# codex-storage/codex-storage-proofs-circuits

Hardware: AMD Instinct MI355X
Metric: Poseidon2-BN254 permutations/sec per GPU; full proof-input witnesses/sec (higher is better)
Workload: dtype u32x9 (29-bit limbs, Montgomery mod BN254 r)

## Files before the change

### codex-storage-proofs-circuits_amd/csrc/proof_many.cpp

```cpp
#include <hip/hip_runtime.h>

#include <fcntl.h>
#include <unistd.h>

#include <algorithm>
#include <cstring>
#include <map>
#include <memory>
#include <string>
#include <vector>

#include "dataset_obj.hpp"
#include "proof_input_obj.hpp"
#include "trees.hpp"

using namespace cp2i;

namespace {

struct Req {
  cp2_dataset* ds = nullptr;
  uint64_t slot = 0;
  uint8_t entropy[32];
  size_t at = 0;
  size_t id = 0;
};

int refuse(cp2_ctx* ctx, size_t i, const std::string& why) {
  ctx->err = "request " + std::to_string(i) + ": " + why;
  return CP2_ERR_INVALID;
}

size_t depth_of(size_t n) { return layer_sizes_of(n).size() - 1; }

bool same_circuit(const cp2_config& a, const cp2_config& b) {
  return a.max_depth == b.max_depth && a.max_log2_nslots == b.max_log2_nslots && a.cell_size == b.cell_size && a.block_size == b.block_size &&
         a.n_samples == b.n_samples;
}

int validate(cp2_ctx* ctx, cp2_dataset* const* ds, const uint64_t* slot_idx, size_t n) {
  for (size_t i = 0; i < n; ++i) {
    const cp2_dataset* d = ds[i];
    if (!d) return refuse(ctx, i, "NULL dataset");
    if (d->ctx != ctx) return refuse(ctx, i, "its dataset belongs to another context");
    const cp2_config& c = d->cfg;
    if (!same_circuit(c, ds[0]->cfg))
      return refuse(ctx, i, "its circuit parameters (maxDepth, maxLog2NSlots, cellSize, blockSize, nSamples) differ from request 0's");
    const uint64_t s = slot_idx[i];
    if (s < d->first_slot || s - d->first_slot >= d->n_local)
      return refuse(ctx, i, "slot " + std::to_string(s) + " is not local to its dataset (slots " + std::to_string(d->first_slot) + " .. " +
                                std::to_string(d->first_slot + d->n_local - 1) + ")");
    if (!d->have_roots && !(d->first_slot == 0 && d->n_local == c.n_slots))
      return refuse(ctx, i, "its dataset has no dataset tree: not all of its slots are local and cp2_dataset_set_roots was never called");
    if (!is_pow2(c.n_cells) || (c.n_samples && c.n_cells < 2))
      return refuse(ctx, i, "nCells " + std::to_string(c.n_cells) + " is not a power of two >= 2");
    const size_t cpb = c.block_size / c.cell_size;
    if (depth_of(cpb) + depth_of(c.n_cells / cpb) > (size_t)c.max_depth)
      return refuse(ctx, i, "its slot tree is deeper than maxDepth");
    if (depth_of(c.n_slots) > (size_t)c.max_log2_nslots)
      return refuse(ctx, i, "its dataset tree is deeper than maxLog2NSlots");
    if (!d->trees && d->tree_mode == 2 && d->csizes.size() - 1 != depth_of(c.n_cells / cpb))
      return refuse(ctx, i, "its compact layers do not match its configuration");
  }
  return CP2_OK;
}

int check_roots(cp2_ctx* ctx, cp2_dataset* const* ds, const uint64_t* slot_idx, size_t n) {
  std::vector<uint64_t> a(n);
  for (size_t i = 0; i < n; ++i)
    a[i] = (uint64_t)reinterpret_cast<uintptr_t>(dataset_roots_dev(ds[i])) + (slot_idx[i] - ds[i]->first_slot) * 32;
  std::vector<uint8_t> got(n * 32);
  DevBuf d_a, d_r;
  CP2_TRY(d_a.scratch(ctx, n * 8));
  CP2_TRY(d_r.scratch(ctx, n * 32));
  CP2_HIP(ctx, hipMemcpyAsync(d_a.p, a.data(), n * 8, hipMemcpyHostToDevice, ctx->stream));
  CP2_HIP(ctx, cp2k::launch_gather_addr(static_cast<const uint64_t*>(d_a.p), n, 32, d_r.p, ctx->stream));
  CP2_HIP(ctx, hipMemcpyAsync(got.data(), d_r.p, n * 32, hipMemcpyDeviceToHost, ctx->stream));
  CP2_HIP(ctx, hipStreamSynchronize(ctx->stream));
  for (size_t i = 0; i < n; ++i)
    if (std::memcmp(&got[i * 32], &ds[i]->dlayers[slot_idx[i] * 32], 32) != 0)
      return refuse(ctx, i, "the root its dataset tree holds for slot " + std::to_string(slot_idx[i]) +
                                " (cp2_dataset_set_roots) differs from the slot's built root");
  return CP2_OK;
}

int prepare(cp2_ctx* ctx, cp2_dataset* const* ds, const uint64_t* slot_idx, size_t n) {
  CP2_TRY(validate(ctx, ds, slot_idx, n));
  CP2_HIP(ctx, hipSetDevice(ctx->device));
  for (size_t i = 0; i < n; ++i)
    if (!ds[i]->have_roots) CP2_TRY(cp2_dataset_set_roots(ds[i], nullptr));
  return check_roots(ctx, ds, slot_idx, n);
}

std::string who(bool named, const Req* r) { return named ? "request " + std::to_string(r->id) + ": " : std::string(); }

int run_pass(cp2_ctx* ctx, const std::vector<const Req*>& rq, size_t n_rf, size_t n_rfile, size_t n_cf, bool named, cp2_proof_input** out) {
  const size_t n = rq.size(), nr = n_rf + n_rfile;
  const cp2_config& c0 = rq[0]->ds->cfg;
  const size_t ns = c0.n_samples, md = (size_t)c0.max_depth, cs = c0.cell_size, bs = c0.block_size, cpb = bs / cs;
  const size_t T = n * ns, R = nr * ns, C = T - R, RF = n_rf * ns, CF = n_cf * ns;
  auto store = std::make_shared<BatchStore>();
  if (T) {
    std::vector<cp2k::ManyReq> reqs(n);
    std::vector<cp2k::TreeGeom> geoms;
    std::map<std::string, uint32_t> geom_of;
    for (size_t j = 0; j < n; ++j) {
      const cp2_dataset* ds = rq[j]->ds;
      cp2k::ManyReq& q = reqs[j];
      std::memset(&q, 0, sizeof q);
      std::memcpy(q.entropy, rq[j]->entropy, 32);
      std::memcpy(q.slot_root, &ds->dlayers[rq[j]->slot * 32], 32);
      q.n_cells = ds->cfg.n_cells;
      q.cpb = cpb;
      if (j < nr) {
        cp2k::TreeGeom g;
        std::memset(&g, 0, sizeof g);
        trees_geom(ds->trees, &g);
        auto it = geom_of.emplace(std::string(reinterpret_cast<const char*>(&g), sizeof g), (uint32_t)geoms.size());
        if (it.second) geoms.push_back(g);
        q.geom = it.first->second;
        q.nodes = (uint64_t)reinterpret_cast<uintptr_t>(ds->trees->nodes.p);
        q.slot = rq[j]->slot - ds->first_slot;
      }
    }
    std::vector<uint64_t> blk(C), gen, cpaths, ctail, ccell;
    std::vector<uint8_t> checks(2 * C * 32);
    PinBuf h_blocks;
    const size_t rows = T * md + T + 2 * C;
    DevBuf d_req, d_geom, d_idx, d_blk, d_addr, d_rows, d_cells, d_gen, d_caddr;
    CP2_TRY(d_req.scratch(ctx, n * sizeof(cp2k::ManyReq)));
    CP2_TRY(d_geom.scratch(ctx, std::max<size_t>(1, geoms.size()) * sizeof(cp2k::TreeGeom)));
    CP2_TRY(d_idx.scratch(ctx, T * 8));
    CP2_TRY(d_blk.scratch(ctx, T * 8));
    CP2_TRY(d_addr.scratch(ctx, rows * 8));
    CP2_TRY(d_rows.scratch(ctx, rows * 32));
    CP2_TRY(d_cells.scratch(ctx, (C * cpb + T) * cs));
    CP2_TRY(store->idx.alloc(ctx, T * 8));
    CP2_TRY(store->paths.alloc(ctx, T * md * 32));
    CP2_TRY(store->leaves.alloc(ctx, T * 32));
    CP2_TRY(store->cells.alloc(ctx, T * cs));
    uint8_t* cells_out = d_cells.u8() + C * cpb * cs;
    uint64_t* addr = static_cast<uint64_t*>(d_addr.p);
    CP2_HIP(ctx, hipMemcpyAsync(d_req.p, reqs.data(), n * sizeof(cp2k::ManyReq), hipMemcpyHostToDevice, ctx->stream));
    if (!geoms.empty())
      CP2_HIP(ctx, hipMemcpyAsync(d_geom.p, geoms.data(), geoms.size() * sizeof(cp2k::TreeGeom), hipMemcpyHostToDevice, ctx->stream));
    CP2_HIP(ctx, cp2k::launch_sample_many(static_cast<const cp2k::ManyReq*>(d_req.p), static_cast<const cp2k::TreeGeom*>(d_geom.p), n,
                                          (uint32_t)ns, (uint32_t)md, static_cast<uint64_t*>(d_idx.p), static_cast<uint64_t*>(d_blk.p), addr,
                                          ctx->stream));
    CP2_HIP(ctx, hipMemcpyAsync(store->idx.p, d_idx.p, T * 8, hipMemcpyDeviceToHost, ctx->stream));
    if (C) CP2_HIP(ctx, hipMemcpyAsync(blk.data(), static_cast<uint64_t*>(d_blk.p) + R, C * 8, hipMemcpyDeviceToHost, ctx->stream));
    CP2_HIP(ctx, hipStreamSynchronize(ctx->stream));
    const uint64_t* idx = static_cast<const uint64_t*>(store->idx.p);

    gen.assign((CF + RF) * 2, 0);
    uint64_t* seeds = gen.data();
    uint64_t* firsts = seeds + CF + RF;
    for (size_t q = 0; q < CF; ++q) {
      const Req* r = rq[nr + q / ns];
      seeds[q] = cp2_slot_seed(r->ds->cfg.seed, r->slot);
      firsts[q] = blk[q] * cpb;
    }
    for (size_t p = 0; p < RF; ++p) {
      const Req* r = rq[p / ns];
      seeds[CF + p] = cp2_slot_seed(r->ds->cfg.seed, r->slot);
      firsts[CF + p] = idx[p];
    }
    if (CF + RF) {
      CP2_TRY(d_gen.scratch(ctx, gen.size() * 8));
      const uint64_t* dg = static_cast<const uint64_t*>(d_gen.p);
      CP2_HIP(ctx, hipMemcpyAsync(d_gen.p, gen.data(), gen.size() * 8, hipMemcpyHostToDevice, ctx->stream));
      CP2_HIP(ctx, cp2k::launch_gen_fake_cells_many(dg, dg + CF + RF, cpb, CF * cpb, cs, d_cells.p, ctx->stream));
      CP2_HIP(ctx, cp2k::launch_gen_fake_cells_many(dg + CF, dg + CF + RF + CF, 1, RF, cs, cells_out, ctx->stream));
    }
    if (C > CF) {
      const size_t n_req_file = (C - CF) / ns;
      CP2_TRY(h_blocks.alloc(ctx, (C - CF) * bs));
      std::vector<std::string> failed(fill_threads(ctx));
      on_threads(fill_threads(ctx), n_req_file, [&](int w, size_t k) {
        const size_t q0 = CF + k * ns;
        const Req* r = rq[nr + q0 / ns];
        const std::string fname = slot_file_name(r->ds->file_base, r->slot);
        const int fd = open(fname.c_str(), O_RDONLY);
        if (fd < 0) { failed[w] = who(named, r) + "slot " + std::to_string(r->slot) + ": " + slot_file_error(fname, 0); return false; }
        int err = 0;
        size_t c = 0;
        for (; c < ns && !err; ++c) err = slot_file_read_rest(fd, h_blocks.u8() + (q0 - CF + c) * bs, bs, blk[q0 + c] * bs);
        close(fd);
        if (err) {
          failed[w] = who(named, r) + "block " + std::to_string(blk[q0 + c - 1]) + " of slot " + std::to_string(r->slot) +
                      ": " + slot_file_error(fname, err);
          return false;
        }
        return true;
      });
      for (const auto& f : failed)
        if (!f.empty()) { ctx->err = f; return CP2_ERR_IO; }
      CP2_HIP(ctx, hipMemcpyAsync(d_cells.u8() + CF * bs, h_blocks.p, (C - CF) * bs, hipMemcpyHostToDevice, ctx->stream));
    }
    cp2_slot_trees* mini = nullptr;
    struct Mini { cp2_slot_trees*& t; ~Mini() { cp2_slot_trees_free(t); } } mini_guard{mini};
    if (C) {
      cpaths.assign(C * md, 0);
      ctail.assign(3 * C, 0);
      ccell.assign(C, 0);
      CP2_TRY(cp2_slot_trees_build_dev(ctx, d_cells.p, C, cs, bs, cpb, &mini));
      const size_t depth_b = depth_of(cpb);
      const uint64_t mb = (uint64_t)reinterpret_cast<uintptr_t>(mini->nodes.p);
      std::vector<uint64_t> rr(depth_b + 1);
      for (size_t q = 0; q < C; ++q) {
        const Req* r = rq[nr + q / ns];
        const cp2_dataset* ds = r->ds;
        const uint64_t ls = r->slot - ds->first_slot, cell = idx[R + q], b = blk[q], in_block = cell % cpb;
        const uint64_t kb = (uint64_t)reinterpret_cast<uintptr_t>(ds->compact.p);
        uint64_t* P = &cpaths[q * md];
        path_rows(mini, q, in_block, depth_b + 1, rr.data());
        for (size_t d = 0; d < depth_b; ++d) P[d] = rr[d] == NO_ROW ? 0 : mb + rr[d] * 32;
        uint64_t j = b, m = ds->cfg.n_cells / cpb;
        for (size_t d = 0; d + 1 < ds->csizes.size(); ++d) {
          const uint64_t sib = j ^ 1;
          P[depth_b + d] = sib < m ? kb + (ds->coff[d] + ls * ds->csizes[d] + sib) * 32 : 0;
          j >>= 1;
          m = (m + 1) >> 1;
        }
        ctail[q] = mb + (q * cpb + in_block) * 32;
        ctail[C + 2 * q] = kb + (ds->coff[0] + ls * ds->csizes[0] + b) * 32;
        ctail[C + 2 * q + 1] = mb + (mini->toff[0] + q) * 32;
        ccell[q] = (uint64_t)reinterpret_cast<uintptr_t>(d_cells.u8()) + (q * cpb + in_block) * cs;
      }
      CP2_TRY(d_caddr.scratch(ctx, C * 8));
      CP2_HIP(ctx, hipMemcpyAsync(addr + R * md, cpaths.data(), C * md * 8, hipMemcpyHostToDevice, ctx->stream));
      CP2_HIP(ctx, hipMemcpyAsync(addr + T * md + R, ctail.data(), 3 * C * 8, hipMemcpyHostToDevice, ctx->stream));
      CP2_HIP(ctx, hipMemcpyAsync(d_caddr.p, ccell.data(), C * 8, hipMemcpyHostToDevice, ctx->stream));
      CP2_HIP(ctx, cp2k::launch_gather_addr(static_cast<const uint64_t*>(d_caddr.p), C, cs, cells_out + R * cs, ctx->stream));
    }
    CP2_HIP(ctx, cp2k::launch_gather_addr(addr, rows, 32, d_rows.p, ctx->stream));
    CP2_HIP(ctx, hipMemcpyAsync(store->paths.p, d_rows.p, T * md * 32, hipMemcpyDeviceToHost, ctx->stream));
    CP2_HIP(ctx, hipMemcpyAsync(store->leaves.p, d_rows.u8() + T * md * 32, T * 32, hipMemcpyDeviceToHost, ctx->stream));
    if (C) CP2_HIP(ctx, hipMemcpyAsync(checks.data(), d_rows.u8() + (T * md + T) * 32, 2 * C * 32, hipMemcpyDeviceToHost, ctx->stream));
    CP2_HIP(ctx, hipMemcpyAsync(store->cells.p, cells_out, T * cs, hipMemcpyDeviceToHost, ctx->stream));
    CP2_HIP(ctx, hipStreamSynchronize(ctx->stream));
    for (size_t q = 0; q < C; ++q)
      if (std::memcmp(&checks[2 * q * 32], &checks[(2 * q + 1) * 32], 32) != 0) {
        const Req* r = rq[nr + q / ns];
        ctx->err = who(named, r) + "block " + std::to_string(blk[q]) + " of slot " + std::to_string(r->slot) +
                   " does not hash to its stored root (slot data changed since the build?)";
        return CP2_ERR_IO;
      }
    if (R > RF) {
      std::vector<std::string> failed(fill_threads(ctx));
      on_threads(fill_threads(ctx), n_rfile, [&](int w, size_t k) {
        const Req* r = rq[n_rf + k];
        const std::string fname = slot_file_name(r->ds->file_base, r->slot);
        const int fd = open(fname.c_str(), O_RDONLY);
        if (fd < 0) { failed[w] = who(named, r) + slot_file_error(fname, 0); return false; }
        int err = 0;
        const size_t p0 = (n_rf + k) * ns;
        for (size_t c = 0; c < ns && !err; ++c) err = read_file_cell(fd, cs, idx[p0 + c], store->cells.u8() + (p0 + c) * cs);
        close(fd);
        if (err) { failed[w] = who(named, r) + slot_file_error(fname, err); return false; }
        return true;
      });
      for (const auto& f : failed)
        if (!f.empty()) { ctx->err = f; return CP2_ERR_IO; }
    }
  }
  std::vector<ProofItem> items(n);
  for (size_t j = 0; j < n; ++j) items[j] = {rq[j]->ds, rq[j]->slot, rq[j]->entropy, &out[rq[j]->at]};
  return proof_inputs_from_store(items.data(), n, store, store->cells.u8());
}

}

int cp2i::prove_requests(cp2_ctx* ctx, cp2_dataset* const* ds, const uint64_t* slot_idx, const uint8_t* entropies, size_t n, size_t at0,
                         bool named, cp2_proof_input** out) {
  for (size_t i = 0; i < n; ++i) out[i] = nullptr;
  if (n == 0) return CP2_OK;
  CP2_HIP(ctx, hipSetDevice(ctx->device));
  std::vector<Req> req(n);
  std::vector<const Req*> res_fake, res_file, cmp_fake, cmp_file, roots_only;
  for (size_t i = 0; i < n; ++i) {
    req[i].ds = ds[i];
    req[i].slot = slot_idx[i];
    req[i].at = i;
    req[i].id = at0 + i;
    canonical_felt(entropies + 32 * i, req[i].entropy);
    const cp2_dataset* d = ds[i];
    (d->trees ? (d->from_file ? res_file : res_fake) : d->tree_mode == 2 ? (d->from_file ? cmp_file : cmp_fake) : roots_only).push_back(&req[i]);
  }
  auto fail = [&](int st) {
    for (size_t i = 0; i < n; ++i) { cp2_proof_input_free(out[i]); out[i] = nullptr; }
    return st;
  };
  for (const Req* r : roots_only) {
    const int st = cp2_proof_inputs_generate_batch(r->ds, &r->slot, 1, r->entropy, &out[r->at]);
    if (st != CP2_OK) {
      ctx->err = who(named, r) + ctx->err;
      return fail(st);
    }
  }
  const cp2_config& c0 = ds[0]->cfg;
  const size_t per_req = std::max<size_t>(1, (size_t)c0.n_samples * c0.block_size);
  const size_t chunk = std::max<size_t>(1, ctx->stage_bytes / per_req);
  std::vector<const Req*> compact(cmp_fake);
  compact.insert(compact.end(), cmp_file.begin(), cmp_file.end());
  const size_t n_res = res_fake.size() + res_file.size();
  size_t c = 0;
  for (bool first = true; first ? n_res + compact.size() > 0 : c < compact.size(); first = false) {
    std::vector<const Req*> rq;
    if (first) {
      rq = res_fake;
      rq.insert(rq.end(), res_file.begin(), res_file.end());
    }
    const size_t c1 = std::min(compact.size(), c + chunk);
    rq.insert(rq.end(), compact.begin() + (long)c, compact.begin() + (long)c1);
    const size_t n_cf = c < cmp_fake.size() ? std::min(c1, cmp_fake.size()) - c : 0;
    const int st = run_pass(ctx, rq, first ? res_fake.size() : 0, first ? res_file.size() : 0, n_cf, named, out);
    if (st != CP2_OK) return fail(st);
    c = c1;
  }
  return CP2_OK;
}

extern "C" int cp2_proof_inputs_generate_many(cp2_ctx* ctx, cp2_dataset* const* ds, const uint64_t* slot_idx, const uint8_t* entropies, size_t n,
                                              cp2_proof_input** out) try {
  if (!ctx) return CP2_ERR_INVALID;
  if (n && (!ds || !slot_idx || !entropies || !out)) {
    ctx->err = "cp2_proof_inputs_generate_many: NULL array";
    return CP2_ERR_INVALID;
  }
  for (size_t i = 0; i < n; ++i) out[i] = nullptr;
  if (n == 0) return CP2_OK;
  CP2_REFUSE_STUCK(ctx);
  CP2_TRY(prepare(ctx, ds, slot_idx, n));
  return prove_requests(ctx, ds, slot_idx, entropies, n, 0, true, out);
} catch (const std::bad_alloc&) {
  return CP2_ERR_ALLOC;
} catch (...) {
  return CP2_ERR_INVALID;
}

extern "C" int cp2_proof_inputs_export_many(cp2_ctx* ctx, cp2_dataset* const* ds, const uint64_t* slot_idx, const uint8_t* entropies, size_t n,
                                            const char* const* paths, int threads, size_t batch, uint64_t* total_bytes) try {
  if (!ctx) return CP2_ERR_INVALID;
  if (n && (!ds || !slot_idx || !entropies)) {
    ctx->err = "cp2_proof_inputs_export_many: NULL array";
    return CP2_ERR_INVALID;
  }
  if (total_bytes) *total_bytes = 0;
  if (n == 0) return CP2_OK;
  CP2_REFUSE_STUCK(ctx);
  CP2_TRY(prepare(ctx, ds, slot_idx, n));
  if (batch == 0) batch = 512;
  if (threads < 1) threads = 1;
  uint64_t bytes = 0;
  int status = CP2_OK;
  std::vector<cp2_proof_input*> cur, next;
  auto generate = [&](size_t b0, std::vector<cp2_proof_input*>& o) -> int {
    const size_t m = std::min(batch, n - b0);
    o.assign(m, nullptr);
    return prove_requests(ctx, ds + b0, slot_idx + b0, entropies + 32 * b0, m, b0, true, o.data());
  };
  struct Release {
    std::vector<cp2_proof_input*>& v;
    ~Release() { for (auto* p : v) cp2_proof_input_free(p); v.clear(); }
  } rel_cur{cur}, rel_next{next};
  status = generate(0, cur);
  for (size_t b0 = 0; status == CP2_OK && b0 < n; b0 += batch) {
    const size_t b1 = b0 + batch;
    int gen_status = CP2_OK, st = CP2_OK;
    uint64_t got = 0;
    {
      Workers producer(1);
      if (b1 < n) producer.submit([&] { gen_status = generate(b1, next); });
      st = cp2_proof_inputs_write_json_batch(cur.data(), cur.size(), paths ? paths + b0 : nullptr, threads, &got);
    }
    bytes += got;
    for (auto* p : cur) cp2_proof_input_free(p);
    cur.clear();
    if (st != CP2_OK) status = st;
    else if (gen_status != CP2_OK) status = gen_status;
    cur.swap(next);
  }
  if (total_bytes) *total_bytes = bytes;
  return status;
} catch (const std::bad_alloc&) {
  return CP2_ERR_ALLOC;
} catch (...) {
  return CP2_ERR_INVALID;
}
```

Measured before the change: 767.1 million.

## Deduplicate touched blocks per request and double-buffer compact proof passes

Sampling now runs once for all requests. A per-request hash table then deduplicates the blocks each compact request touches, so every distinct block is read, generated and hashed only once, and pass sizing follows the distinct-block count. Passes use two preallocated device and pinned buffer sets so the host work for the next pass (file reads, path assembly) overlaps the current pass's GPU work. The cost is more code, larger and more complex buffer management, and a fallback to a single buffer set when allocation fails.

```diff
diff --git a/codex-storage-proofs-circuits_amd/csrc/proof_many.cpp b/codex-storage-proofs-circuits_amd/csrc/proof_many.cpp
--- a/codex-storage-proofs-circuits_amd/csrc/proof_many.cpp
+++ b/codex-storage-proofs-circuits_amd/csrc/proof_many.cpp
@@ -4,6 +4,9 @@
 #include <unistd.h>
 
 #include <algorithm>
+#include <chrono>
+#include <cstdio>
+#include <cstdlib>
 #include <cstring>
 #include <map>
 #include <memory>
@@ -12,6 +15,7 @@
 
 #include "dataset_obj.hpp"
 #include "proof_input_obj.hpp"
+#include "touched_plan.hpp"
 #include "trees.hpp"
 
 using namespace cp2i;
@@ -94,180 +98,313 @@
 
 std::string who(bool named, const Req* r) { return named ? "request " + std::to_string(r->id) + ": " : std::string(); }
 
-int run_pass(cp2_ctx* ctx, const std::vector<const Req*>& rq, size_t n_rf, size_t n_rfile, size_t n_cf, bool named, cp2_proof_input** out) {
-  const size_t n = rq.size(), nr = n_rf + n_rfile;
-  const cp2_config& c0 = rq[0]->ds->cfg;
-  const size_t ns = c0.n_samples, md = (size_t)c0.max_depth, cs = c0.cell_size, bs = c0.block_size, cpb = bs / cs;
-  const size_t T = n * ns, R = nr * ns, C = T - R, RF = n_rf * ns, CF = n_cf * ns;
-  auto store = std::make_shared<BatchStore>();
-  if (T) {
-    std::vector<cp2k::ManyReq> reqs(n);
-    std::vector<cp2k::TreeGeom> geoms;
-    std::map<std::string, uint32_t> geom_of;
-    for (size_t j = 0; j < n; ++j) {
-      const cp2_dataset* ds = rq[j]->ds;
-      cp2k::ManyReq& q = reqs[j];
-      std::memset(&q, 0, sizeof q);
-      std::memcpy(q.entropy, rq[j]->entropy, 32);
-      std::memcpy(q.slot_root, &ds->dlayers[rq[j]->slot * 32], 32);
-      q.n_cells = ds->cfg.n_cells;
-      q.cpb = cpb;
-      if (j < nr) {
-        cp2k::TreeGeom g;
-        std::memset(&g, 0, sizeof g);
-        trees_geom(ds->trees, &g);
-        auto it = geom_of.emplace(std::string(reinterpret_cast<const char*>(&g), sizeof g), (uint32_t)geoms.size());
-        if (it.second) geoms.push_back(g);
-        q.geom = it.first->second;
-        q.nodes = (uint64_t)reinterpret_cast<uintptr_t>(ds->trees->nodes.p);
-        q.slot = rq[j]->slot - ds->first_slot;
+struct PassDims {
+  size_t r0 = 0, r1 = 0;
+  size_t R = 0, RF = 0;
+  size_t C = 0;
+  size_t d0 = 0, D = 0, DF = 0;
+};
+
+struct PassLayout {
+  size_t n_rows = 0, root_row = 0, node_rows = 0;
+  size_t addr = 0, rows = 0, cells = 0, nodes = 0, gen = 0, caddr = 0, dev_bytes = 0;
+  size_t h_addr = 0, h_gen = 0, h_caddr = 0, h_checks = 0, h_blocks = 0, pin_bytes = 0;
+};
+
+size_t carve(size_t& off, size_t bytes) {
+  const size_t at = off;
+  off += (bytes + 255) & ~(size_t)255;
+  return at;
+}
+
+struct PassSet {
+  DevBuf dev;
+  PinBuf pin;
+  hipEvent_t done = nullptr;
+  ~PassSet() { if (done) (void)hipEventDestroy(done); }
+};
+
+struct Pass {
+  PassDims d;
+  PassLayout l;
+  std::shared_ptr<BatchStore> store;
+};
+
+struct Call {
+  cp2_ctx* ctx = nullptr;
+  bool named = false;
+  cp2_proof_input** out = nullptr;
+  std::vector<const Req*> rq;
+  size_t n_rf = 0, n_rfile = 0, n_cf = 0, n_cfile = 0;
+  size_t ns = 0, md = 0, cs = 0, bs = 0, cpb = 0;
+  std::vector<size_t> bsizes;
+  size_t per_block = 0;
+  size_t R_all = 0, C_all = 0;
+  DevBuf dev;
+  PinBuf pin;
+  uint64_t* d_raddr = nullptr;
+  uint8_t* d_rrows = nullptr;
+  const uint64_t* idx = nullptr;
+  const uint64_t* blk = nullptr;
+  TouchedPlan plan;
+  PassSet sets[2];
+  size_t nr() const { return n_rf + n_rfile; }
+  const Req* compact_req(size_t r) const { return rq[nr() + r]; }
+};
+
+PassLayout layout_of(const Call& c, const PassDims& d) {
+  PassLayout l;
+  const size_t T = d.R + d.C;
+  l.n_rows = d.C * c.md + d.C + 2 * d.D;
+  l.root_row = d.D * c.per_block;
+  l.node_rows = l.root_row + d.D;
+  size_t off = 0;
+  l.addr = carve(off, l.n_rows * 8);
+  l.rows = carve(off, l.n_rows * 32);
+  l.cells = carve(off, (d.D * c.cpb + T) * c.cs);
+  l.nodes = carve(off, l.node_rows * 32);
+  l.gen = carve(off, 2 * (d.DF + d.RF) * 8);
+  l.caddr = carve(off, d.C * 8);
+  l.dev_bytes = off;
+  off = 0;
+  l.h_addr = carve(off, l.n_rows * 8);
+  l.h_gen = carve(off, 2 * (d.DF + d.RF) * 8);
+  l.h_caddr = carve(off, d.C * 8);
+  l.h_checks = carve(off, 2 * d.D * 32);
+  l.h_blocks = carve(off, (d.D - d.DF) * c.bs);
+  l.pin_bytes = off;
+  return l;
+}
+
+int sample_all(Call& c) {
+  cp2_ctx* ctx = c.ctx;
+  const size_t n = c.rq.size(), nr = c.nr(), T_all = c.R_all + c.C_all, raddr_rows = c.R_all * c.md + c.R_all;
+  std::vector<cp2k::TreeGeom> geoms;
+  std::map<std::string, uint32_t> geom_of;
+  size_t off = 0;
+  const size_t o_req = carve(off, n * sizeof(cp2k::ManyReq)), o_idx = carve(off, T_all * 8), o_blk = carve(off, c.C_all * 8);
+  CP2_TRY(c.pin.alloc(ctx, off));
+  cp2k::ManyReq* reqs = reinterpret_cast<cp2k::ManyReq*>(c.pin.u8() + o_req);
+  for (size_t j = 0; j < n; ++j) {
+    const cp2_dataset* ds = c.rq[j]->ds;
+    cp2k::ManyReq& q = reqs[j];
+    std::memset(&q, 0, sizeof q);
+    std::memcpy(q.entropy, c.rq[j]->entropy, 32);
+    std::memcpy(q.slot_root, &ds->dlayers[c.rq[j]->slot * 32], 32);
+    q.n_cells = ds->cfg.n_cells;
+    q.cpb = c.cpb;
+    if (j < nr) {
+      cp2k::TreeGeom g;
+      std::memset(&g, 0, sizeof g);
+      trees_geom(ds->trees, &g);
+      auto it = geom_of.emplace(std::string(reinterpret_cast<const char*>(&g), sizeof g), (uint32_t)geoms.size());
+      if (it.second) geoms.push_back(g);
+      q.geom = it.first->second;
+      q.nodes = (uint64_t)reinterpret_cast<uintptr_t>(ds->trees->nodes.p);
+      q.slot = c.rq[j]->slot - ds->first_slot;
+    }
+  }
+  size_t doff = 0;
+  const size_t d_req = carve(doff, n * sizeof(cp2k::ManyReq)), d_geom = carve(doff, geoms.size() * sizeof(cp2k::TreeGeom)),
+               d_idx = carve(doff, T_all * 8), d_blk = carve(doff, c.C_all * 8), d_raddr = carve(doff, raddr_rows * 8),
+               d_rrows = carve(doff, raddr_rows * 32);
+  CP2_TRY(c.dev.scratch(ctx, doff));
+  uint8_t* base = c.dev.u8();
+  c.d_raddr = reinterpret_cast<uint64_t*>(base + d_raddr);
+  c.d_rrows = base + d_rrows;
+  const cp2k::ManyReq* dreq = reinterpret_cast<const cp2k::ManyReq*>(base + d_req);
+  uint64_t* didx = reinterpret_cast<uint64_t*>(base + d_idx);
+  CP2_HIP(ctx, hipMemcpyAsync(base + d_req, reqs, n * sizeof(cp2k::ManyReq), hipMemcpyHostToDevice, ctx->stream));
+  if (!geoms.empty())
+    CP2_HIP(ctx, hipMemcpyAsync(base + d_geom, geoms.data(), geoms.size() * sizeof(cp2k::TreeGeom), hipMemcpyHostToDevice, ctx->stream));
+  CP2_HIP(ctx, cp2k::launch_sample_many(dreq, reinterpret_cast<const cp2k::TreeGeom*>(base + d_geom), nr, (uint32_t)c.ns, (uint32_t)c.md, didx,
+                                        nullptr, c.d_raddr, ctx->stream));
+  CP2_HIP(ctx, cp2k::launch_sample_many(dreq + nr, nullptr, n - nr, (uint32_t)c.ns, (uint32_t)c.md, didx + c.R_all,
+                                        reinterpret_cast<uint64_t*>(base + d_blk), nullptr, ctx->stream));
+  if (T_all) CP2_HIP(ctx, hipMemcpyAsync(c.pin.u8() + o_idx, didx, T_all * 8, hipMemcpyDeviceToHost, ctx->stream));
+  if (c.C_all) CP2_HIP(ctx, hipMemcpyAsync(c.pin.u8() + o_blk, base + d_blk, c.C_all * 8, hipMemcpyDeviceToHost, ctx->stream));
+  CP2_HIP(ctx, hipStreamSynchronize(ctx->stream));
+  c.idx = reinterpret_cast<const uint64_t*>(c.pin.u8() + o_idx);
+  c.blk = reinterpret_cast<const uint64_t*>(c.pin.u8() + o_blk);
+  const size_t cap_blocks = ctx->stage_bytes / c.bs;
+  const size_t chunk = std::max<size_t>(1, ctx->stage_bytes / std::max<size_t>(1, c.ns * c.bs));
+  c.plan = touched_plan(c.blk, c.n_cf + c.n_cfile, c.ns, cap_blocks, 4 * chunk);
+  return CP2_OK;
+}
+
+int enqueue_pass(Call& c, Pass& p, PassSet& set) {
+  cp2_ctx* ctx = c.ctx;
+  const PassDims& d = p.d;
+  const PassLayout& l = p.l;
+  const size_t ns = c.ns, md = c.md, cs = c.cs, bs = c.bs, cpb = c.cpb, T = d.R + d.C;
+  uint8_t* dev = set.dev.u8();
+  uint8_t* pin = set.pin.u8();
+  uint8_t* d_cells = dev + l.cells;
+  uint8_t* cells_out = d_cells + d.D * cpb * cs;
+  uint8_t* d_rows = dev + l.rows;
+  uint64_t* d_addr = reinterpret_cast<uint64_t*>(dev + l.addr);
+  p.store = std::make_shared<BatchStore>();
+  CP2_TRY(p.store->idx.alloc(ctx, T * 8));
+  CP2_TRY(p.store->paths.alloc(ctx, T * md * 32));
+  CP2_TRY(p.store->leaves.alloc(ctx, T * 32));
+  CP2_TRY(p.store->cells.alloc(ctx, T * cs));
+  uint64_t* sidx = static_cast<uint64_t*>(p.store->idx.p);
+  std::memcpy(sidx, c.idx, d.R * 8);
+  std::memcpy(sidx + d.R, c.idx + c.R_all + d.r0 * ns, d.C * 8);
+  if (d.DF + d.RF) {
+    uint64_t* seeds = reinterpret_cast<uint64_t*>(pin + l.h_gen);
+    uint64_t* firsts = seeds + d.DF + d.RF;
+    for (size_t r = d.r0, k = 0; r < d.r1 && r < c.n_cf; ++r) {
+      const Req* rq = c.compact_req(r);
+      const uint64_t seed = cp2_slot_seed(rq->ds->cfg.seed, rq->slot);
+      for (size_t g = c.plan.first[r]; g < c.plan.first[r + 1]; ++g, ++k) {
+        seeds[k] = seed;
+        firsts[k] = c.plan.block[g] * cpb;
       }
     }
-    std::vector<uint64_t> blk(C), gen, cpaths, ctail, ccell;
-    std::vector<uint8_t> checks(2 * C * 32);
-    PinBuf h_blocks;
-    const size_t rows = T * md + T + 2 * C;
-    DevBuf d_req, d_geom, d_idx, d_blk, d_addr, d_rows, d_cells, d_gen, d_caddr;
-    CP2_TRY(d_req.scratch(ctx, n * sizeof(cp2k::ManyReq)));
-    CP2_TRY(d_geom.scratch(ctx, std::max<size_t>(1, geoms.size()) * sizeof(cp2k::TreeGeom)));
-    CP2_TRY(d_idx.scratch(ctx, T * 8));
-    CP2_TRY(d_blk.scratch(ctx, T * 8));
-    CP2_TRY(d_addr.scratch(ctx, rows * 8));
-    CP2_TRY(d_rows.scratch(ctx, rows * 32));
-    CP2_TRY(d_cells.scratch(ctx, (C * cpb + T) * cs));
-    CP2_TRY(store->idx.alloc(ctx, T * 8));
-    CP2_TRY(store->paths.alloc(ctx, T * md * 32));
-    CP2_TRY(store->leaves.alloc(ctx, T * 32));
-    CP2_TRY(store->cells.alloc(ctx, T * cs));
-    uint8_t* cells_out = d_cells.u8() + C * cpb * cs;
-    uint64_t* addr = static_cast<uint64_t*>(d_addr.p);
-    CP2_HIP(ctx, hipMemcpyAsync(d_req.p, reqs.data(), n * sizeof(cp2k::ManyReq), hipMemcpyHostToDevice, ctx->stream));
-    if (!geoms.empty())
-      CP2_HIP(ctx, hipMemcpyAsync(d_geom.p, geoms.data(), geoms.size() * sizeof(cp2k::TreeGeom), hipMemcpyHostToDevice, ctx->stream));
-    CP2_HIP(ctx, cp2k::launch_sample_many(static_cast<const cp2k::ManyReq*>(d_req.p), static_cast<const cp2k::TreeGeom*>(d_geom.p), n,
-                                          (uint32_t)ns, (uint32_t)md, static_cast<uint64_t*>(d_idx.p), static_cast<uint64_t*>(d_blk.p), addr,
-                                          ctx->stream));
-    CP2_HIP(ctx, hipMemcpyAsync(store->idx.p, d_idx.p, T * 8, hipMemcpyDeviceToHost, ctx->stream));
-    if (C) CP2_HIP(ctx, hipMemcpyAsync(blk.data(), static_cast<uint64_t*>(d_blk.p) + R, C * 8, hipMemcpyDeviceToHost, ctx->stream));
-    CP2_HIP(ctx, hipStreamSynchronize(ctx->stream));
-    const uint64_t* idx = static_cast<const uint64_t*>(store->idx.p);
-
-    gen.assign((CF + RF) * 2, 0);
-    uint64_t* seeds = gen.data();
-    uint64_t* firsts = seeds + CF + RF;
-    for (size_t q = 0; q < CF; ++q) {
-      const Req* r = rq[nr + q / ns];
-      seeds[q] = cp2_slot_seed(r->ds->cfg.seed, r->slot);
-      firsts[q] = blk[q] * cpb;
-    }
-    for (size_t p = 0; p < RF; ++p) {
-      const Req* r = rq[p / ns];
-      seeds[CF + p] = cp2_slot_seed(r->ds->cfg.seed, r->slot);
-      firsts[CF + p] = idx[p];
-    }
-    if (CF + RF) {
-      CP2_TRY(d_gen.scratch(ctx, gen.size() * 8));
-      const uint64_t* dg = static_cast<const uint64_t*>(d_gen.p);
-      CP2_HIP(ctx, hipMemcpyAsync(d_gen.p, gen.data(), gen.size() * 8, hipMemcpyHostToDevice, ctx->stream));
-      CP2_HIP(ctx, cp2k::launch_gen_fake_cells_many(dg, dg + CF + RF, cpb, CF * cpb, cs, d_cells.p, ctx->stream));
-      CP2_HIP(ctx, cp2k::launch_gen_fake_cells_many(dg + CF, dg + CF + RF + CF, 1, RF, cs, cells_out, ctx->stream));
-    }
-    if (C > CF) {
-      const size_t n_req_file = (C - CF) / ns;
-      CP2_TRY(h_blocks.alloc(ctx, (C - CF) * bs));
-      std::vector<std::string> failed(fill_threads(ctx));
-      on_threads(fill_threads(ctx), n_req_file, [&](int w, size_t k) {
-        const size_t q0 = CF + k * ns;
-        const Req* r = rq[nr + q0 / ns];
-        const std::string fname = slot_file_name(r->ds->file_base, r->slot);
-        const int fd = open(fname.c_str(), O_RDONLY);
-        if (fd < 0) { failed[w] = who(named, r) + "slot " + std::to_string(r->slot) + ": " + slot_file_error(fname, 0); return false; }
-        int err = 0;
-        size_t c = 0;
-        for (; c < ns && !err; ++c) err = slot_file_read_rest(fd, h_blocks.u8() + (q0 - CF + c) * bs, bs, blk[q0 + c] * bs);
-        close(fd);
-        if (err) {
-          failed[w] = who(named, r) + "block " + std::to_string(blk[q0 + c - 1]) + " of slot " + std::to_string(r->slot) +
-                      ": " + slot_file_error(fname, err);
-          return false;
-        }
-        return true;
-      });
-      for (const auto& f : failed)
-        if (!f.empty()) { ctx->err = f; return CP2_ERR_IO; }
-      CP2_HIP(ctx, hipMemcpyAsync(d_cells.u8() + CF * bs, h_blocks.p, (C - CF) * bs, hipMemcpyHostToDevice, ctx->stream));
-    }
-    cp2_slot_trees* mini = nullptr;
-    struct Mini { cp2_slot_trees*& t; ~Mini() { cp2_slot_trees_free(t); } } mini_guard{mini};
-    if (C) {
-      cpaths.assign(C * md, 0);
-      ctail.assign(3 * C, 0);
-      ccell.assign(C, 0);
-      CP2_TRY(cp2_slot_trees_build_dev(ctx, d_cells.p, C, cs, bs, cpb, &mini));
-      const size_t depth_b = depth_of(cpb);
-      const uint64_t mb = (uint64_t)reinterpret_cast<uintptr_t>(mini->nodes.p);
-      std::vector<uint64_t> rr(depth_b + 1);
-      for (size_t q = 0; q < C; ++q) {
-        const Req* r = rq[nr + q / ns];
-        const cp2_dataset* ds = r->ds;
-        const uint64_t ls = r->slot - ds->first_slot, cell = idx[R + q], b = blk[q], in_block = cell % cpb;
-        const uint64_t kb = (uint64_t)reinterpret_cast<uintptr_t>(ds->compact.p);
-        uint64_t* P = &cpaths[q * md];
-        path_rows(mini, q, in_block, depth_b + 1, rr.data());
-        for (size_t d = 0; d < depth_b; ++d) P[d] = rr[d] == NO_ROW ? 0 : mb + rr[d] * 32;
-        uint64_t j = b, m = ds->cfg.n_cells / cpb;
-        for (size_t d = 0; d + 1 < ds->csizes.size(); ++d) {
+    for (size_t q = 0; q < d.RF; ++q) {
+      const Req* rq = c.rq[q / ns];
+      seeds[d.DF + q] = cp2_slot_seed(rq->ds->cfg.seed, rq->slot);
+      firsts[d.DF + q] = c.idx[q];
+    }
+    const uint64_t* dg = reinterpret_cast<const uint64_t*>(dev + l.gen);
+    CP2_HIP(ctx, hipMemcpyAsync(dev + l.gen, seeds, 2 * (d.DF + d.RF) * 8, hipMemcpyHostToDevice, ctx->stream));
+    CP2_HIP(ctx, cp2k::launch_gen_fake_cells_many(dg, dg + d.DF + d.RF, cpb, d.DF * cpb, cs, d_cells, ctx->stream));
+    CP2_HIP(ctx, cp2k::launch_gen_fake_cells_many(dg + d.DF, dg + d.DF + d.RF + d.DF, 1, d.RF, cs, cells_out, ctx->stream));
+  }
+  if (d.D > d.DF) {
+    const size_t f0 = std::max(d.r0, c.n_cf), g0 = d.d0 + d.DF;
+    uint8_t* h_blocks = pin + l.h_blocks;
+    std::vector<std::string> failed(fill_threads(ctx));
+    on_threads(fill_threads(ctx), d.r1 - f0, [&](int w, size_t k) {
+      const size_t r = f0 + k;
+      const Req* rq = c.compact_req(r);
+      const std::string fname = slot_file_name(rq->ds->file_base, rq->slot);
+      const int fd = open(fname.c_str(), O_RDONLY);
+      if (fd < 0) { failed[w] = who(c.named, rq) + "slot " + std::to_string(rq->slot) + ": " + slot_file_error(fname, 0); return false; }
+      int err = 0;
+      size_t g = c.plan.first[r];
+      for (; g < c.plan.first[r + 1] && !err; ++g) err = slot_file_read_rest(fd, h_blocks + (g - g0) * bs, bs, c.plan.block[g] * bs);
+      close(fd);
+      if (err) {
+        failed[w] = who(c.named, rq) + "block " + std::to_string(c.plan.block[g - 1]) + " of slot " + std::to_string(rq->slot) +
+                    ": " + slot_file_error(fname, err);
+        return false;
+      }
+      return true;
+    });
+    for (const auto& f : failed)
+      if (!f.empty()) { ctx->err = f; return CP2_ERR_IO; }
+    CP2_HIP(ctx, hipMemcpyAsync(d_cells + d.DF * bs, h_blocks, (d.D - d.DF) * bs, hipMemcpyHostToDevice, ctx->stream));
+  }
+  if (d.D) {
+    uint8_t* nodes = dev + l.nodes;
+    const uint64_t mb = (uint64_t)reinterpret_cast<uintptr_t>(nodes);
+    const size_t nb = c.bsizes.size(), depth_b = nb - 1;
+    std::vector<size_t> boff(nb, 0);
+    for (size_t k = 1; k < nb; ++k) boff[k] = boff[k - 1] + d.D * c.bsizes[k - 1];
+    CP2_HIP(ctx, cp2k::launch_hash_cells(d_cells, cs, d.D * cpb, nodes, ctx->stream));
+    for (size_t k = 0; k + 1 < nb; ++k)
+      CP2_HIP(ctx, cp2k::launch_compress_layer(nodes + boff[k] * 32, nodes + boff[k + 1] * 32, c.bsizes[k], d.D, k == 0, c.bsizes[k],
+                                               c.bsizes[k + 1], ctx->stream));
+    uint64_t* h_addr = reinterpret_cast<uint64_t*>(pin + l.h_addr);
+    uint64_t* h_leaf = h_addr + d.C * md;
+    uint64_t* h_check = h_leaf + d.C;
+    uint64_t* h_caddr = reinterpret_cast<uint64_t*>(pin + l.h_caddr);
+    std::memset(h_addr, 0, d.C * md * 8);
+    for (size_t r = d.r0; r < d.r1; ++r) {
+      const Req* rq = c.compact_req(r);
+      const cp2_dataset* ds = rq->ds;
+      const uint64_t ls = rq->slot - ds->first_slot, kb = (uint64_t)reinterpret_cast<uintptr_t>(ds->compact.p);
+      for (size_t g = c.plan.first[r]; g < c.plan.first[r + 1]; ++g) {
+        h_check[2 * (g - d.d0)] = kb + (ds->coff[0] + ls * ds->csizes[0] + c.plan.block[g]) * 32;
+        h_check[2 * (g - d.d0) + 1] = mb + (boff[depth_b] + (g - d.d0)) * 32;
+      }
+      for (size_t s = 0; s < ns; ++s) {
+        const size_t lane = r * ns + s, q = lane - d.r0 * ns, g = c.plan.lane_pair[lane] - d.d0;
+        const uint64_t cell = c.idx[c.R_all + lane], b = c.blk[lane], in_block = cell % cpb;
+        uint64_t* P = h_addr + q * md;
+        uint64_t j = in_block, m = cpb;
+        for (size_t k = 0; k < depth_b; ++k) {
           const uint64_t sib = j ^ 1;
-          P[depth_b + d] = sib < m ? kb + (ds->coff[d] + ls * ds->csizes[d] + sib) * 32 : 0;
+          P[k] = sib < m ? mb + (boff[k] + g * c.bsizes[k] + sib) * 32 : 0;
           j >>= 1;
           m = (m + 1) >> 1;
         }
-        ctail[q] = mb + (q * cpb + in_block) * 32;
-        ctail[C + 2 * q] = kb + (ds->coff[0] + ls * ds->csizes[0] + b) * 32;
-        ctail[C + 2 * q + 1] = mb + (mini->toff[0] + q) * 32;
-        ccell[q] = (uint64_t)reinterpret_cast<uintptr_t>(d_cells.u8()) + (q * cpb + in_block) * cs;
+        j = b;
+        m = ds->cfg.n_cells / cpb;
+        for (size_t k = 0; k + 1 < ds->csizes.size(); ++k) {
+          const uint64_t sib = j ^ 1;
+          P[depth_b + k] = sib < m ? kb + (ds->coff[k] + ls * ds->csizes[k] + sib) * 32 : 0;
+          j >>= 1;
+          m = (m + 1) >> 1;
+        }
+        h_leaf[q] = mb + (g * cpb + in_block) * 32;
+        h_caddr[q] = (uint64_t)reinterpret_cast<uintptr_t>(d_cells) + (g * cpb + in_block) * cs;
       }
-      CP2_TRY(d_caddr.scratch(ctx, C * 8));
-      CP2_HIP(ctx, hipMemcpyAsync(addr + R * md, cpaths.data(), C * md * 8, hipMemcpyHostToDevice, ctx->stream));
-      CP2_HIP(ctx, hipMemcpyAsync(addr + T * md + R, ctail.data(), 3 * C * 8, hipMemcpyHostToDevice, ctx->stream));
-      CP2_HIP(ctx, hipMemcpyAsync(d_caddr.p, ccell.data(), C * 8, hipMemcpyHostToDevice, ctx->stream));
-      CP2_HIP(ctx, cp2k::launch_gather_addr(static_cast<const uint64_t*>(d_caddr.p), C, cs, cells_out + R * cs, ctx->stream));
-    }
-    CP2_HIP(ctx, cp2k::launch_gather_addr(addr, rows, 32, d_rows.p, ctx->stream));
-    CP2_HIP(ctx, hipMemcpyAsync(store->paths.p, d_rows.p, T * md * 32, hipMemcpyDeviceToHost, ctx->stream));
-    CP2_HIP(ctx, hipMemcpyAsync(store->leaves.p, d_rows.u8() + T * md * 32, T * 32, hipMemcpyDeviceToHost, ctx->stream));
-    if (C) CP2_HIP(ctx, hipMemcpyAsync(checks.data(), d_rows.u8() + (T * md + T) * 32, 2 * C * 32, hipMemcpyDeviceToHost, ctx->stream));
-    CP2_HIP(ctx, hipMemcpyAsync(store->cells.p, cells_out, T * cs, hipMemcpyDeviceToHost, ctx->stream));
-    CP2_HIP(ctx, hipStreamSynchronize(ctx->stream));
-    for (size_t q = 0; q < C; ++q)
-      if (std::memcmp(&checks[2 * q * 32], &checks[(2 * q + 1) * 32], 32) != 0) {
-        const Req* r = rq[nr + q / ns];
-        ctx->err = who(named, r) + "block " + std::to_string(blk[q]) + " of slot " + std::to_string(r->slot) +
+    }
+    CP2_HIP(ctx, hipMemcpyAsync(d_addr, h_addr, l.n_rows * 8, hipMemcpyHostToDevice, ctx->stream));
+    CP2_HIP(ctx, hipMemcpyAsync(dev + l.caddr, h_caddr, d.C * 8, hipMemcpyHostToDevice, ctx->stream));
+    CP2_HIP(ctx, cp2k::launch_gather_addr(reinterpret_cast<const uint64_t*>(dev + l.caddr), d.C, cs, cells_out + d.R * cs, ctx->stream));
+    CP2_HIP(ctx, cp2k::launch_gather_addr(d_addr, l.n_rows, 32, d_rows, ctx->stream));
+    CP2_HIP(ctx, hipMemcpyAsync(p.store->paths.u8() + d.R * md * 32, d_rows, d.C * md * 32, hipMemcpyDeviceToHost, ctx->stream));
+    CP2_HIP(ctx, hipMemcpyAsync(p.store->leaves.u8() + d.R * 32, d_rows + d.C * md * 32, d.C * 32, hipMemcpyDeviceToHost, ctx->stream));
+    CP2_HIP(ctx, hipMemcpyAsync(pin + l.h_checks, d_rows + (d.C * md + d.C) * 32, 2 * d.D * 32, hipMemcpyDeviceToHost, ctx->stream));
+  }
+  if (d.R) {
+    CP2_HIP(ctx, cp2k::launch_gather_addr(c.d_raddr, d.R * md + d.R, 32, c.d_rrows, ctx->stream));
+    CP2_HIP(ctx, hipMemcpyAsync(p.store->paths.p, c.d_rrows, d.R * md * 32, hipMemcpyDeviceToHost, ctx->stream));
+    CP2_HIP(ctx, hipMemcpyAsync(p.store->leaves.p, c.d_rrows + d.R * md * 32, d.R * 32, hipMemcpyDeviceToHost, ctx->stream));
+  }
+  if (T) CP2_HIP(ctx, hipMemcpyAsync(p.store->cells.p, cells_out, T * cs, hipMemcpyDeviceToHost, ctx->stream));
+  CP2_HIP(ctx, hipEventRecord(set.done, ctx->stream));
+  return CP2_OK;
+}
+
+int finish_pass(Call& c, Pass& p, PassSet& set) {
+  cp2_ctx* ctx = c.ctx;
+  const PassDims& d = p.d;
+  CP2_HIP(ctx, hipEventSynchronize(set.done));
+  const uint8_t* checks = set.pin.u8() + p.l.h_checks;
+  for (size_t r = d.r0; r < d.r1; ++r)
+    for (size_t g = c.plan.first[r]; g < c.plan.first[r + 1]; ++g)
+      if (std::memcmp(checks + 2 * (g - d.d0) * 32, checks + (2 * (g - d.d0) + 1) * 32, 32) != 0) {
+        const Req* rq = c.compact_req(r);
+        ctx->err = who(c.named, rq) + "block " + std::to_string(c.plan.block[g]) + " of slot " + std::to_string(rq->slot) +
                    " does not hash to its stored root (slot data changed since the build?)";
         return CP2_ERR_IO;
       }
-    if (R > RF) {
-      std::vector<std::string> failed(fill_threads(ctx));
-      on_threads(fill_threads(ctx), n_rfile, [&](int w, size_t k) {
-        const Req* r = rq[n_rf + k];
-        const std::string fname = slot_file_name(r->ds->file_base, r->slot);
-        const int fd = open(fname.c_str(), O_RDONLY);
-        if (fd < 0) { failed[w] = who(named, r) + slot_file_error(fname, 0); return false; }
-        int err = 0;
-        const size_t p0 = (n_rf + k) * ns;
-        for (size_t c = 0; c < ns && !err; ++c) err = read_file_cell(fd, cs, idx[p0 + c], store->cells.u8() + (p0 + c) * cs);
-        close(fd);
-        if (err) { failed[w] = who(named, r) + slot_file_error(fname, err); return false; }
-        return true;
-      });
-      for (const auto& f : failed)
-        if (!f.empty()) { ctx->err = f; return CP2_ERR_IO; }
-    }
-  }
-  std::vector<ProofItem> items(n);
-  for (size_t j = 0; j < n; ++j) items[j] = {rq[j]->ds, rq[j]->slot, rq[j]->entropy, &out[rq[j]->at]};
-  return proof_inputs_from_store(items.data(), n, store, store->cells.u8());
-}
+  if (d.R > d.RF) {
+    const size_t ns = c.ns, cs = c.cs;
+    std::vector<std::string> failed(fill_threads(ctx));
+    on_threads(fill_threads(ctx), c.n_rfile, [&](int w, size_t k) {
+      const Req* rq = c.rq[c.n_rf + k];
+      const std::string fname = slot_file_name(rq->ds->file_base, rq->slot);
+      const int fd = open(fname.c_str(), O_RDONLY);
+      if (fd < 0) { failed[w] = who(c.named, rq) + slot_file_error(fname, 0); return false; }
+      int err = 0;
+      const size_t p0 = (c.n_rf + k) * ns;
+      for (size_t s = 0; s < ns && !err; ++s) err = read_file_cell(fd, cs, c.idx[p0 + s], p.store->cells.u8() + (p0 + s) * cs);
+      close(fd);
+      if (err) { failed[w] = who(c.named, rq) + slot_file_error(fname, err); return false; }
+      return true;
+    });
+    for (const auto& f : failed)
+      if (!f.empty()) { ctx->err = f; return CP2_ERR_IO; }
+  }
+  std::vector<ProofItem> items;
+  auto item = [&](const Req* rq) { items.push_back({rq->ds, rq->slot, rq->entropy, &c.out[rq->at]}); };
+  for (size_t j = 0; j < d.R / std::max<size_t>(1, c.ns); ++j) item(c.rq[j]);
+  for (size_t r = d.r0; r < d.r1; ++r) item(c.compact_req(r));
+  return proof_inputs_from_store(items.data(), items.size(), p.store, p.store->cells.u8());
+}
+
+struct Drain {
+  cp2_ctx* ctx;
+  ~Drain() { if (!ctx->stuck) (void)hipStreamSynchronize(ctx->stream); }
+};
+
+double now_s() { return std::chrono::duration<double>(std::chrono::steady_clock::now().time_since_epoch()).count(); }
 
 }
 
@@ -275,6 +412,7 @@
                          bool named, cp2_proof_input** out) {
   for (size_t i = 0; i < n; ++i) out[i] = nullptr;
   if (n == 0) return CP2_OK;
+  const double t0 = now_s();
   CP2_HIP(ctx, hipSetDevice(ctx->device));
   std::vector<Req> req(n);
   std::vector<const Req*> res_fake, res_file, cmp_fake, cmp_file, roots_only;
@@ -298,26 +436,103 @@
       return fail(st);
     }
   }
+  Call c;
+  c.ctx = ctx;
+  c.named = named;
+  c.out = out;
+  c.n_rf = res_fake.size();
+  c.n_rfile = res_file.size();
+  c.n_cf = cmp_fake.size();
+  c.n_cfile = cmp_file.size();
+  for (const auto* v : {&res_fake, &res_file, &cmp_fake, &cmp_file}) c.rq.insert(c.rq.end(), v->begin(), v->end());
+  if (c.rq.empty()) return CP2_OK;
   const cp2_config& c0 = ds[0]->cfg;
-  const size_t per_req = std::max<size_t>(1, (size_t)c0.n_samples * c0.block_size);
-  const size_t chunk = std::max<size_t>(1, ctx->stage_bytes / per_req);
-  std::vector<const Req*> compact(cmp_fake);
-  compact.insert(compact.end(), cmp_file.begin(), cmp_file.end());
-  const size_t n_res = res_fake.size() + res_file.size();
-  size_t c = 0;
-  for (bool first = true; first ? n_res + compact.size() > 0 : c < compact.size(); first = false) {
-    std::vector<const Req*> rq;
-    if (first) {
-      rq = res_fake;
-      rq.insert(rq.end(), res_file.begin(), res_file.end());
-    }
-    const size_t c1 = std::min(compact.size(), c + chunk);
-    rq.insert(rq.end(), compact.begin() + (long)c, compact.begin() + (long)c1);
-    const size_t n_cf = c < cmp_fake.size() ? std::min(c1, cmp_fake.size()) - c : 0;
-    const int st = run_pass(ctx, rq, first ? res_fake.size() : 0, first ? res_file.size() : 0, n_cf, named, out);
-    if (st != CP2_OK) return fail(st);
-    c = c1;
-  }
+  c.ns = c0.n_samples;
+  c.md = (size_t)c0.max_depth;
+  c.cs = c0.cell_size;
+  c.bs = c0.block_size;
+  c.cpb = c.bs / c.cs;
+  c.bsizes = layer_sizes_of(c.cpb);
+  for (size_t k = 0; k + 1 < c.bsizes.size(); ++k) c.per_block += c.bsizes[k];
+  c.R_all = c.nr() * c.ns;
+  c.C_all = (c.n_cf + c.n_cfile) * c.ns;
+  std::vector<Pass> passes;
+  Drain drain{ctx};
+  if (c.R_all + c.C_all == 0) {
+    auto store = std::make_shared<BatchStore>();
+    std::vector<ProofItem> items;
+    for (const Req* r : c.rq) items.push_back({r->ds, r->slot, r->entropy, &out[r->at]});
+    const int st = proof_inputs_from_store(items.data(), items.size(), store, store->cells.u8());
+    return st == CP2_OK ? st : fail(st);
+  }
+  int st = sample_all(c);
+  if (st != CP2_OK) return fail(st);
+  const size_t np = std::max<size_t>(1, c.plan.passes());
+  passes.resize(np);
+  size_t dev_bytes = 0, pin_bytes = 0;
+  for (size_t k = 0; k < np; ++k) {
+    PassDims& d = passes[k].d;
+    if (c.plan.passes()) {
+      d.r0 = c.plan.pass_first[k];
+      d.r1 = c.plan.pass_first[k + 1];
+    }
+    d.C = (d.r1 - d.r0) * c.ns;
+    d.d0 = c.plan.first[d.r0];
+    d.D = c.plan.first[d.r1] - d.d0;
+    d.DF = d.r0 < c.n_cf ? c.plan.first[std::min(d.r1, c.n_cf)] - d.d0 : 0;
+    if (k == 0) {
+      d.R = c.R_all;
+      d.RF = c.n_rf * c.ns;
+    }
+    passes[k].l = layout_of(c, d);
+    dev_bytes = std::max(dev_bytes, passes[k].l.dev_bytes);
+    pin_bytes = std::max(pin_bytes, passes[k].l.pin_bytes);
+  }
+  int n_sets = 0;
+  for (int s = 0; s < (np > 1 ? 2 : 1); ++s) {
+    PassSet& set = c.sets[s];
+    int got = set.dev.scratch(ctx, dev_bytes);
+    if (got == CP2_OK) got = set.pin.alloc(ctx, pin_bytes);
+    if (got == CP2_OK && hipEventCreateWithFlags(&set.done, hipEventDisableTiming) != hipSuccess) {
+      (void)hipGetLastError();
+      set.done = nullptr;
+      ctx->err = "hipEventCreateWithFlags failed";
+      got = CP2_ERR_HIP;
+    }
+    if (got != CP2_OK) {
+      if (s == 0) return fail(got);
+      set.dev.release();
+      set.pin.release();
+      ctx->err.clear();
+      break;
+    }
+    ++n_sets;
+  }
+  if (n_sets == 2) {
+    st = enqueue_pass(c, passes[0], c.sets[0]);
+    for (size_t k = 0; k < np && st == CP2_OK; ++k) {
+      int st_next = CP2_OK;
+      std::string err_next;
+      if (k + 1 < np) {
+        st_next = enqueue_pass(c, passes[k + 1], c.sets[(k + 1) & 1]);
+        if (st_next != CP2_OK) err_next = ctx->err;
+      }
+      st = finish_pass(c, passes[k], c.sets[k & 1]);
+      if (st == CP2_OK && st_next != CP2_OK) {
+        ctx->err = err_next;
+        st = st_next;
+      }
+    }
+  } else {
+    for (size_t k = 0; k < np && st == CP2_OK; ++k) {
+      st = enqueue_pass(c, passes[k], c.sets[0]);
+      if (st == CP2_OK) st = finish_pass(c, passes[k], c.sets[0]);
+    }
+  }
+  if (st != CP2_OK) return fail(st);
+  if (std::getenv("CP2_TRACE"))
+    std::fprintf(stderr, "[cp2 trace] prove_requests: requests=%zu compact=%zu lanes=%zu distinct_blocks=%zu passes=%zu sets=%d seconds=%.6f\n",
+                 c.rq.size(), c.n_cf + c.n_cfile, c.C_all, c.plan.block.size(), np, n_sets, now_s() - t0);
   return CP2_OK;
 }
 
diff --git a/codex-storage-proofs-circuits_amd/csrc/touched_plan.hpp b/codex-storage-proofs-circuits_amd/csrc/touched_plan.hpp
--- /dev/null
+++ b/codex-storage-proofs-circuits_amd/csrc/touched_plan.hpp
@@ -0,0 +1,57 @@
+#pragma once
+#include <cstddef>
+#include <cstdint>
+#include <vector>
+
+namespace cp2i {
+
+struct TouchedPlan {
+  std::vector<uint64_t> block;
+  std::vector<size_t> first, lane_pair, pass_first;
+  size_t passes() const { return pass_first.empty() ? 0 : pass_first.size() - 1; }
+  size_t pairs_of_pass(size_t k) const { return first[pass_first[k + 1]] - first[pass_first[k]]; }
+};
+
+inline TouchedPlan touched_plan(const uint64_t* lane_block, size_t n_req, size_t n_samples, size_t cap_blocks, size_t max_requests) {
+  TouchedPlan p;
+  p.first.assign(n_req + 1, 0);
+  p.lane_pair.assign(n_req * n_samples, 0);
+  p.block.reserve(n_req * n_samples);
+  size_t tab = 4;
+  while (tab < 2 * n_samples) tab <<= 1;
+  std::vector<uint64_t> key(tab);
+  std::vector<size_t> val(tab), stamp(tab, 0);
+  for (size_t r = 0; r < n_req; ++r) {
+    p.first[r] = p.block.size();
+    for (size_t c = 0; c < n_samples; ++c) {
+      const size_t q = r * n_samples + c;
+      const uint64_t b = lane_block[q];
+      size_t h = (size_t)((b * 0x9e3779b97f4a7c15ULL) >> 17) & (tab - 1);
+      while (stamp[h] == r + 1 && key[h] != b) h = (h + 1) & (tab - 1);
+      if (stamp[h] != r + 1) {
+        stamp[h] = r + 1;
+        key[h] = b;
+        val[h] = p.block.size();
+        p.block.push_back(b);
+      }
+      p.lane_pair[q] = val[h];
+    }
+  }
+  p.first[n_req] = p.block.size();
+  if (n_req == 0) return p;
+  p.pass_first.push_back(0);
+  size_t held = 0, reqs = 0;
+  for (size_t r = 0; r < n_req; ++r) {
+    const size_t own = p.first[r + 1] - p.first[r];
+    if (reqs && (held + own > cap_blocks || (max_requests && reqs == max_requests))) {
+      p.pass_first.push_back(r);
+      held = reqs = 0;
+    }
+    held += own;
+    ++reqs;
+  }
+  p.pass_first.push_back(n_req);
+  return p;
+}
+
+}
```

Result: no change. 768.0 million (median of 4 runs) (+0.1%).
